# kartikmadhira1/YA_VO

Hardware: AMD Instinct MI355X
Metric: frames/sec (detect+describe+match+PnP) on 1241×376 KITTI stereo; RMSE vs CPU ref (higher is better)
Workload: dtype u8

## Files before the change

include/yavo/yavo.h:

```cpp
#ifndef YAVO_H
#define YAVO_H

#include <stddef.h>
#include <stdint.h>

#include "yavo_types.h"

#ifdef __cplusplus
extern "C" {
#endif

#define YV_OK 0
#define YV_ERR_INVALID (-1)
#define YV_ERR_HIP (-2)
#define YV_ERR_NODEVICE (-3)
#define YV_ERR_CAPACITY (-4)

#define YV_ABI_VERSION 2

typedef struct yv_ctx yv_ctx;
typedef struct yv_batch yv_batch;

int yv_abi_version(void);
const char* yv_status_string(int status);
// ... 73 lines not shown
int yv_batch_orient_view_get(yv_batch* b, yv_batch_orient_view* v);
int yv_batch_set_match_gates(yv_batch* b, const int32_t* gates , int n_pairs);
int yv_batch_set_stereo_subpix(yv_batch* b, const int32_t* pair_idx , int n, int half_win, int search,
                               int flags);
typedef struct yv_batch_subpix_view {
    const int32_t* dcol_q8;
    const int32_t* sad;
    const uint8_t* status;
} yv_batch_subpix_view;
int yv_batch_subpix_view_get(yv_batch* b, yv_batch_subpix_view* v);
int yv_batch_set_tracks(yv_batch* b, const int32_t* tracks , int n_tracks, const double K[9],
                        const double T_right[7]);
int yv_batch_track(yv_batch* b, const double* d_priors, double* d_poses, void* stream);
int yv_batch_set_track_overlap(yv_batch* b, int on);
int yv_batch_track_sync(yv_batch* b);
int yv_batch_set_track_lk(yv_batch* b, int image_step, int win, int max_level, int max_count, double eps,
                          double min_eig);
int yv_batch_enable_timing(yv_batch* b, int on);
int yv_batch_stage_times(yv_batch* b, float* ms , int* n_runs);
#define YV_NUM_STAGES 7

typedef struct yv_batch_view {
    int max_images, max_kp, max_pairs, H, W;
    int64_t cand_cap;
    const uint32_t* cand_count;
    const int32_t* det_count;
    const int32_t* det_rc;
    const float* det_resp;
    const int32_t* kp_count;
    const yv_keypoint* keypoints;
// ... 26 lines not shown
```

ya_vo_amd/__init__.py:

```python
from __future__ import annotations

import atexit
import ctypes
import os
import weakref
from typing import Optional, Tuple

import numpy as np

_HERE = os.path.dirname(os.path.abspath(__file__))
LIB_PATH = os.environ.get("YAVO_LIB") or os.path.join(_HERE, "lib", "libyavo.so")

YV_OK = 0
YV_ERR_INVALID = -1
YV_ERR_HIP = -2
YV_ERR_NODEVICE = -3
YV_ERR_CAPACITY = -4
YV_NUM_STAGES = 7
STAGE_NAMES = ("detect", "topk", "brief", "match", "finalize", "track_edges", "track_pose")

KEYPOINT_DTYPE = np.dtype([("x", "<i4"), ("y", "<i4"), ("id", "<i4"), ("matched", "u1"),
                           ("featVec", "u1", (32,)), ("_pad", "u1", (3,))])
MATCH_DTYPE = np.dtype([("pt1", KEYPOINT_DTYPE), ("pt2", KEYPOINT_DTYPE), ("distance", "<i4")])
assert KEYPOINT_DTYPE.itemsize == 48 and MATCH_DTYPE.itemsize == 100
# ... 77 lines not shown
    "yv_batch_orient_view_get": (_I, [_P, ctypes.POINTER(_BatchOrientView)]),
    "yv_stereo_subpix": (_I, [_P, _P, _P, _I, _I, _I, _P, _I, _I, _I, _P, _P, _P]),
    "yv_batch_set_stereo_subpix": (_I, [_P, _P, _I, _I, _I, _I]),
    "yv_batch_subpix_view_get": (_I, [_P, ctypes.POINTER(_BatchSubpixView)]),
    "yv_batch_create": (_I, [_P, _I, _I, _I, _I, _I, ctypes.POINTER(_P)]),
    "yv_batch_destroy": (None, [_P]),
    "yv_batch_set_pairs": (_I, [_P, _P, _I]),
    "yv_batch_run": (_I, [_P, _P, _I, _I, ctypes.c_int64, _I, _I, _P]),
    "yv_batch_enable_timing": (_I, [_P, _I]),
    "yv_batch_stage_times": (_I, [_P, _P, ctypes.POINTER(_I)]),
    "yv_batch_view_get": (_I, [_P, ctypes.POINTER(_BatchView)]),
    "yv_batch_set_tracks": (_I, [_P, _P, _I, _P, _P]),
    "yv_batch_track": (_I, [_P, _P, _P, _P]),
    "yv_batch_set_track_overlap": (_I, [_P, _I]),
    "yv_batch_track_sync": (_I, [_P]),
    "yv_batch_set_track_lk": (_I, [_P, _I, _I, _I, _I, ctypes.c_double, ctypes.c_double]),
}


_D = ctypes.c_double
GEOM_SIGNATURES = {
    "yv_f_ransac": (_I, [_P, _P, _I, _P, _I, _D, _P, ctypes.POINTER(_I), ctypes.POINTER(_I)]),
    "yv_triangulate": (_I, [_P, _P, _P, _P, _P, _I, _P, _P, ctypes.POINTER(_I)]),
    "yv_triangulate_subpix": (_I, [_P, _P, _P, _P, _P, _P, _I, _P, _P, ctypes.POINTER(_I)]),
    "yv_world2camera": (_I, [_P, _P, _I, _P, _P, _P]),
    "yv_pose_lm": (_I, [_P, _P, _P, _I, _P, _P, _P, ctypes.POINTER(_I)]),
    "yv_pose_gn": (_I, [_P, _P, _P, _I, _P, _P, ctypes.POINTER(_I)]),
    "yv_pose_lm_batch": (_I, [_P, _I, _P, _P, _P, _P, _P, _P, _P, _P]),
    "yv_pose_gn_batch": (_I, [_P, _I, _P, _P, _P, _P, _P, _P, _P]),
    "yv_f_ransac_batch": (_I, [_P, _P, ctypes.c_int64, _P, _I, _P, ctypes.c_int64, _I, _D, _P, _P, _P, _P]),
# ... 518 lines not shown
    def map_release(self, stream: int) -> None:
        _check(self.lib.yv_batch_map_release(self.handle, ctypes.c_void_p(stream)), "yv_batch_map_release")

    def set_track_overlap(self, on=True) -> None:
        mode = int(on) if not isinstance(on, bool) else (1 if on else 0)
        _check(self.lib.yv_batch_set_track_overlap(self.handle, mode), "yv_batch_set_track_overlap")

    def set_track_lk(self, image_step: int, win: int = 11, max_level: int = 3, max_count: int = 30, eps: float = 0.01,
                     min_eig: float = 0.001) -> None:
        _check(self.lib.yv_batch_set_track_lk(self.handle, image_step, win, max_level, max_count, eps, min_eig),
               "yv_batch_set_track_lk")

    def track_sync(self) -> None:
        _check(self.lib.yv_batch_track_sync(self.handle), "yv_batch_track_sync")

    def enable_timing(self, on=True) -> None:
        mode = 2 if (not isinstance(on, bool) and on == 2) else (1 if on else 0)
        _check(self.lib.yv_batch_enable_timing(self.handle, mode), "yv_batch_enable_timing")

    def stage_times(self) -> Tuple[np.ndarray, int]:
        ms = np.zeros(8, np.float32)
        n = ctypes.c_int()
        _check(self.lib.yv_batch_stage_times(self.handle, _ptr(ms), ctypes.byref(n)), "yv_batch_stage_times")
        return ms[:YV_NUM_STAGES].copy(), n.value

    def view(self) -> _BatchView:
        v = _BatchView()
        _check(self.lib.yv_batch_view_get(self.handle, ctypes.byref(v)), "yv_batch_view_get")
        return v

# ... 266 lines not shown
```

ya_vo_amd/csrc/yavo_api.hip:

```cpp
#include "yavo_host.h"

using namespace yavo;

namespace {

bool in_pinned_scratch(const yv_ctx* ctx, const void* p) {
    const char* c = static_cast<const char*>(p);
    const char* b = reinterpret_cast<const char*>(ctx->h_pinned);
    return ctx->h_pinned && c >= b && c < b + 64 * sizeof(int32_t);
}

}

namespace yavo {

int ctx_device(yv_ctx* ctx) { return ctx->device; }
hipStream_t ctx_stream(yv_ctx* ctx) { return ctx->stream; }

hipError_t stage_sync(yv_ctx* ctx, hipStream_t s) {
    hipError_t e = hipStreamSynchronize(s);
    if (e != hipSuccess) {
        ctx->pending.clear();
        return e;
    }
// ... 154 lines not shown
static int ctx_cus(yv_ctx* ctx) {
    if (ctx->cus <= 0) {
        int cus = 0;
        if (hipDeviceGetAttribute(&cus, hipDeviceAttributeMultiprocessorCount, ctx->device) != hipSuccess || cus <= 0) {
            (void)hipGetLastError();
            cus = 256;
        }
        ctx->cus = cus;
    }
    return ctx->cus;
}

int brief_workers(yv_ctx* ctx, int W) {
    const int w = ctx_cus(ctx) * yavo::brief_workers_per_cu(W);
    return ctx->brief_cap > 0 ? std::min(w, ctx->brief_cap) : w;
}

}

namespace {

int ensure_single(yv_ctx* ctx, int H, int W) {
    if (ctx->single && ctx->single->H == H && ctx->single->W == W) return YV_OK;
    if (ctx->single) {
        batch_free(ctx->single);
        ctx->single = nullptr;
    }
    yv_batch* b = nullptr;
    int rc = yv_batch_create(ctx, 1, H, W, yavo::kMaxKp, 1, &b);
    if (rc != YV_OK) return rc;
// ... 113 lines not shown
    (void)hipSetDevice(ctx->device);
    if (ctx->stream) (void)hipStreamSynchronize(ctx->stream);
    if (ctx->lk_cache) yv_lk_destroy(ctx->lk_cache);
    if (ctx->ess_cache) yv_essential_destroy(ctx->ess_cache);
    batch_free(ctx->single);
    if (ctx->side) (void)hipStreamSynchronize(ctx->side);
    delete ctx;
}

void* yv_stream(yv_ctx* ctx) { return ctx ? reinterpret_cast<void*>(ctx->stream) : nullptr; }

void* yv_side_stream(yv_ctx* ctx) {
    if (!ctx) return nullptr;
    if (ctx->side) return reinterpret_cast<void*>(ctx->side);
    if (set_device(ctx) != YV_OK) return nullptr;
    const int cus = ctx_cus(ctx);
    std::vector<uint32_t> mask((size_t)(cus + 31) / 32, 0u);
    for (int c = 0; c < cus; ++c) mask[(size_t)c / 32] |= 1u << (c % 32);
    if (hipExtStreamCreateWithCUMask(&ctx->side, (uint32_t)mask.size(), mask.data()) != hipSuccess) {
        ctx->side = nullptr;
        (void)hipGetLastError();
        if (hipStreamCreateWithFlags(&ctx->side, hipStreamNonBlocking) != hipSuccess) ctx->side = nullptr;
    }
    if (ctx->side) ctx->mem.adopt(ctx->side);
    return reinterpret_cast<void*>(ctx->side);
}

int yv_sync(yv_ctx* ctx) {
    if (!ctx) return YV_ERR_INVALID;
    YV_HIP(hipStreamSynchronize(ctx->stream));
    return YV_OK;
}

int yv_download(yv_ctx* ctx, void* host_dst, const void* dev_src, size_t bytes) {
    if (!ctx || (bytes > 0 && (!host_dst || !dev_src))) return YV_ERR_INVALID;
    if (bytes == 0) return YV_OK;
    if (set_device(ctx) != YV_OK) return YV_ERR_HIP;
    YV_HIP(hipMemcpyAsync(host_dst, dev_src, bytes, hipMemcpyDeviceToHost, ctx->stream));
// ... 405 lines not shown
```

ya_vo_amd/csrc/yavo_batch.hip:

```cpp
#include "yavo_host.h"

using namespace yavo;

namespace {

constexpr int kMaxTimedRuns = 4096;

int upload_pairs_rev(yv_batch* b) {
    if (!b->m2_alloc || b->n_pairs <= 0) return YV_OK;
    std::vector<int32_t> r(b->h_pairs.size());
    for (size_t i = 0; i + 1 < r.size(); i += 2) {
        r[i] = b->h_pairs[i + 1];
        r[i + 1] = b->h_pairs[i];
    }
    YV_HIP(hipMemcpyAsync(b->pairs_rev, r.data(), sizeof(int32_t) * r.size(), hipMemcpyHostToDevice, b->ctx->stream));
    YV_HIP(hipStreamSynchronize(b->ctx->stream));
    return YV_OK;
}

int record_stage(yv_batch* b, hipStream_t s, int run, int stage) {
    if (!b->timing || run < 0) return YV_OK;
    if (b->timing == 2 && stage > 1) return YV_OK;
    YV_HIP(hipEventRecord(b->events[(size_t)run * kEvPerRun + stage], s));
    return YV_OK;
}

yavo::MatchLists match_lists(const yv_batch* b) { return {b->desc, b->keypoints, b->kp_count, b->max_kp}; }

yavo::MatchRecords match_records(const yv_batch* b) {
    return {b->matches, b->match_count, b->filtered, b->filt_count, b->match_dj, b->match_lim};
}

static_assert(YV_SUBPIX_NONE == yavo::kSubpixNone && YV_SUBPIX_OK == yavo::kSubpixOk &&
                  YV_SUBPIX_OUTSIDE == yavo::kSubpixOutside && YV_SUBPIX_EDGE == yavo::kSubpixEdge,
              "yavo.h / yavo_internal.h");

int subpix_fill_none(yv_batch* b, hipStream_t s) {
    const size_t n = (size_t)std::max(b->max_pairs, 1) * (size_t)b->max_kp;
    YV_HIP(hipMemsetAsync(b->subpix_dcol, 0, n * sizeof(int32_t), s));
    YV_HIP(hipMemsetAsync(b->subpix_sad, 0xFF, n * sizeof(int32_t), s));
    YV_HIP(hipMemsetAsync(b->subpix_status, YV_SUBPIX_NONE, n, s));
    return YV_OK;
}

int ensure_subpix(yv_batch* b) {
// ... 8 lines not shown
        b->mem.release(b->subpix_pairs, b->subpix_dcol, b->subpix_sad, b->subpix_status);
        return YV_ERR_HIP;
    }
    b->subpix_alloc = true;
    return YV_OK;
}

}

namespace yavo {

void batch_free(yv_batch* b) {
    if (!b) return;
    if (b->bstream) (void)hipStreamSynchronize(b->bstream);
    if (b->side) (void)hipStreamSynchronize(b->side);
    if (b->lk) yv_lk_destroy(b->lk);
    delete b;
}

static_assert(YV_MATCH_RATIO == yavo::kMatchRatio && YV_MATCH_MUTUAL == yavo::kMatchMutual, "yavo.h / yavo_internal.h");
static_assert(sizeof(yv_match2) == sizeof(int4), "nn2 is written as int4 {d1, j1, d2, j2}");

bool match_filter_args_ok(int flags, int num, int den) {
    if (flags < 0 || flags > (YV_MATCH_RATIO | YV_MATCH_MUTUAL)) return false;
    if ((flags & YV_MATCH_RATIO) && !(num > 0 && num <= den && den <= 32768)) return false;
    return true;
}

int ensure_match2(yv_batch* b) {
    if (b->m2_alloc) return YV_OK;
// ... 126 lines not shown
    uint32_t* key2 = st.top2 ? b->match_key2 : nullptr;
    if (st.gated) {
        yavo::launch_gate_sort(b->keypoints, b->kp_count, b->nslots, b->max_kp, b->gate_bands, b->gate_cols,
                               b->gate_shift, b->gate_sorted, b->gate_band, s);
        yavo::launch_match_gated(lists, b->pairs, st.n_pairs, b->gate_bands, b->gate_sorted, b->gate_band, b->gates,
                                 false, b->match_key, key2, s);
        if (st.with_rev)
            yavo::launch_match_gated(lists, b->pairs_rev, st.n_pairs, b->gate_bands, b->gate_sorted, b->gate_band,
                                     b->gates, true, b->rev_key, nullptr, s);
    } else {
        yavo::launch_match(lists, b->pairs, st.n_pairs, st.max_train, b->match_key, key2, s);
        if (st.with_rev) yavo::launch_match(lists, b->pairs_rev, st.n_pairs, st.max_train_rev, b->rev_key, nullptr, s);
    }
    const int rc = record_stage(b, s, run, 4);
    const yavo::FinalizeRobust rb{b->match_key2, b->rev_key, st.flags, st.num, st.den, b->nn2, b->rev, b->keep};
    yavo::launch_match_finalize(b->match_key, lists, b->pairs, st.n_pairs, st.thr, match_records(b),
                                st.top2 ? &rb : nullptr, s, st.kp_count_copy, st.n_slots);
    return rc;
}

}

extern "C" {

int yv_batch_create(yv_ctx* ctx, int max_images, int H, int W, int max_kp, int max_pairs, yv_batch** out) {
    if (!ctx || !out || max_images <= 0 || H < 9 || W < 9 || max_kp <= 0 || max_kp > yavo::kMaxKp ||
        max_pairs < 0 || (int64_t)H * W >= (1ll << 31))
        return YV_ERR_INVALID;
    if (W > yavo::kMaxWidth) return YV_ERR_CAPACITY;
    if (H > yavo::kBandRows * yavo::kMaxBands) return YV_ERR_CAPACITY;
    *out = nullptr;
    if (set_device(ctx) != YV_OK) return YV_ERR_HIP;
// ... 59 lines not shown

void yv_batch_destroy(yv_batch* b) {
    if (!b) return;
    (void)hipSetDevice(b->ctx->device);
    (void)hipStreamSynchronize(b->ctx->stream);
    batch_free(b);
}

int yv_batch_set_pairs(yv_batch* b, const int32_t* pairs, int n_pairs) {
    if (!b || n_pairs < 0 || n_pairs > b->max_pairs || (n_pairs > 0 && !pairs)) return YV_ERR_INVALID;
    for (int i = 0; i < 2 * n_pairs; ++i)
        if (pairs[i] < 0 || pairs[i] > b->max_images) return YV_ERR_INVALID;
    if (set_device(b->ctx) != YV_OK) return YV_ERR_HIP;
    if (b->bstream) YV_HIP(hipStreamSynchronize(b->bstream));
    b->build_pending = false;
    if (n_pairs > 0) {
        YV_HIP(hipMemcpyAsync(b->pairs, pairs, sizeof(int32_t) * 2 * (size_t)n_pairs, hipMemcpyHostToDevice,
                              b->ctx->stream));
        YV_HIP(hipStreamSynchronize(b->ctx->stream));
    }
    b->h_pairs.assign(pairs, pairs + 2 * (size_t)n_pairs);
    b->n_pairs = n_pairs;
    b->n_tracks = 0;
    b->gated = false;
    b->subpix_on = false;
    return upload_pairs_rev(b);
}

int yv_batch_set_stereo_subpix(yv_batch* b, const int32_t* pair_idx, int n, int half_win, int search, int flags) {
    if (!b || n < 0) return YV_ERR_INVALID;
// ... 132 lines not shown

int yv_batch_run(yv_batch* b, const uint8_t* d_images, int n_images, int stride, int64_t image_pitch, int match_thr,
                 int carry_from, void* stream) {
    if (!b || !d_images || n_images <= 0 || n_images > b->max_images || stride < b->W ||
        image_pitch < (int64_t)stride * (b->H - 1) + b->W || carry_from >= n_images)
        return YV_ERR_INVALID;
    yv_ctx* ctx = b->ctx;
    if (set_device(ctx) != YV_OK) return YV_ERR_HIP;
    hipStream_t s = stream ? reinterpret_cast<hipStream_t>(stream) : ctx->stream;
    const int H = b->H, W = b->W, K = b->max_kp;
    const int keep = std::min(ctx->max_corners, K);
    const int sel = prepare_select(b, H, W);
    if (sel != YV_OK) return sel;
    const bool steer = steer_on(ctx);
    if (steer && ensure_steer(b) != YV_OK) return YV_ERR_HIP;
    if (b->pending_carry >= 0 && join_build(b, s) != YV_OK) return YV_ERR_HIP;
    if (b->pending_carry >= 0) {
        const size_t c = (size_t)b->pending_carry, dst = (size_t)b->max_images, nk = (size_t)K;
        YV_HIP(hipMemcpyAsync(b->keypoints + dst * nk, b->keypoints + c * nk, nk * sizeof(yv_keypoint),
                              hipMemcpyDeviceToDevice, s));
        YV_HIP(hipMemcpyAsync(b->desc + dst * nk, b->desc + c * nk, nk * sizeof(Desc), hipMemcpyDeviceToDevice, s));
        YV_HIP(hipMemcpyAsync(b->kp_count + dst, b->kp_count + c, sizeof(int32_t), hipMemcpyDeviceToDevice, s));
        if (steer) {
            YV_HIP(hipMemcpyAsync(b->steer_bin + dst * nk, b->steer_bin + c * nk, nk, hipMemcpyDeviceToDevice, s));
            YV_HIP(hipMemcpyAsync(b->steer_mom + dst * nk * 2, b->steer_mom + c * nk * 2, nk * 2 * sizeof(int32_t),
                                  hipMemcpyDeviceToDevice, s));
        }
        b->pending_carry = -1;
    }
    int run = -1;
    if (b->timing && b->runs_recorded < kMaxTimedRuns) run = b->runs_recorded++;
    b->last_run = run;
    int rc = YV_OK;
    rc |= record_stage(b, s, run, 0);
    yavo::launch_detect_blur(d_images, n_images, H, W, stride, image_pitch, ctx->fast_thr, ctx->harris_eigen, b->cand_keys, b->cap,
                             b->cand_count, ctx->k9, b->blur, s);
    rc |= record_stage(b, s, run, 1);
    if (b->overlap_mode == 2) rc |= launch_deferred_after(b, s);
    launch_select_topk(b, n_images, keep, s);
    rc |= record_stage(b, s, run, 2);
    if (b->overlap_mode == 4) rc |= launch_deferred_after(b, s);
    rc |= join_build(b, s);
    launch_describe(b, n_images, brief_workers(ctx, W), s);
    rc |= record_stage(b, s, run, 3);
    if (b->overlap_mode == 3) rc |= launch_deferred_after(b, s);
    b->run_flags = b->n_pairs > 0 ? b->match_flags : 0;
    const bool copy_counts = b->n_pairs > 0 && b->overlap && b->build_async && b->lk_step == 0;
    if (b->n_pairs > 0) {
        MatchStage st;
        st.n_pairs = b->n_pairs;
        st.max_train = st.max_train_rev = K;
        st.top2 = b->run_flags != 0;
        st.with_rev = st.top2 && (b->match_flags & YV_MATCH_MUTUAL) != 0;
        st.gated = b->gated;
        st.thr = match_thr;
        st.flags = b->match_flags;
        st.num = b->ratio_num;
        st.den = b->ratio_den;
        st.kp_count_copy = copy_counts ? b->kp_count_build : nullptr;
        st.n_slots = b->nslots;
        rc |= match_stage(b, st, s, run);
        if (b->subpix_on)
            yavo::launch_subpix_batch(d_images, n_images, H, W, stride, image_pitch, b->subpix_pairs, b->subpix_n,
                                      b->pairs, b->keypoints, b->kp_count, b->match_dj, b->match_lim,
                                      b->run_flags ? b->keep : nullptr, K, b->subpix_win, b->subpix_search,
                                      yavo::SubpixOut{b->subpix_dcol, b->subpix_sad, b->subpix_status}, s);
    } else {
        rc |= record_stage(b, s, run, 4);
    }
    b->counts_copied = copy_counts;
    rc |= record_stage(b, s, run, 5);
    if (rc != YV_OK) return YV_ERR_HIP;
    b->pending_carry = carry_from;
    b->run_images = d_images;
    b->run_n = n_images;
// ... 40 lines not shown
```

ya_vo_amd/csrc/yavo_batch_track.hip:

```cpp
#include "yavo_host.h"

#include <cstdlib>

#include "../../include/yavo/yavo_map.h"

using namespace yavo;

namespace yavo {

int join_build(yv_batch* b, hipStream_t s) {
    if (!b->build_pending) return YV_OK;
    YV_HIP(hipStreamWaitEvent(s, b->ev_built, 0));
    b->build_pending = false;
    return YV_OK;
}

EdgeSlice edge_slice(const yv_batch* b, int k) {
    if (!b->edge_X) return {};
    const size_t nt = (size_t)b->max_tracks, nk = (size_t)b->max_kp;
    return {b->edge_X + k * nt * nk * 3, b->edge_uv + k * nt * nk * 2,  b->edge_query + k * nt * nk,
            b->edge_count + k * nt,      b->edge_outlier + k * nt * nk, b->track_inliers + k * nt};
}

}

namespace {

TrackSrc track_src(const yv_batch* b) {
// ... 146 lines not shown
            const int prev = b->h_pairs[2 * sp];
            if (prev % b->lk_step || prev >= b->max_images || tp < 0 || tp >= b->max_images || tp % b->lk_step)
                return YV_ERR_INVALID;
        } else {
            if (tp < 0 || tp >= b->n_pairs) return YV_ERR_INVALID;
            if (b->h_pairs[2 * sp] != b->h_pairs[2 * tp + 1]) return YV_ERR_INVALID;
        }
    }
    for (int i = 0; i < 9 && n_tracks > 0; ++i)
        if (!std::isfinite(K[i])) return YV_ERR_INVALID;
    if (n_tracks > 0 && !finite_pose(T_right)) return YV_ERR_INVALID;
    if (set_device(b->ctx) != YV_OK) return YV_ERR_HIP;
    hipStream_t s = b->ctx->stream;
    if (b->bstream) YV_HIP(hipStreamSynchronize(b->bstream));
    b->build_pending = false;
    if (b->side) YV_HIP(hipStreamSynchronize(b->side));
    if (n_tracks > b->max_tracks) {
        YV_HIP(hipStreamSynchronize(s));
        if (b->side) YV_HIP(hipStreamSynchronize(b->side));
        b->track_mem.clear();
        b->max_tracks = 0;
        b->n_tracks = 0;
        const size_t nt = (size_t)n_tracks, nk = (size_t)b->max_kp;
        int rc = YV_OK;
        rc |= b->track_mem.alloc(&b->tracks, 2 * nt);
        rc |= b->track_mem.alloc(&b->track_K, 9 * nt);
        rc |= b->track_mem.alloc(&b->T_right, 7);
        rc |= b->track_mem.alloc(&b->edge_X, kEdgeBufs * 3 * nt * nk);
        rc |= b->track_mem.alloc(&b->edge_uv, kEdgeBufs * 2 * nt * nk);
        rc |= b->track_mem.alloc(&b->edge_query, kEdgeBufs * nt * nk);
// ... 70 lines not shown
    if (set_device(b->ctx) != YV_OK) return YV_ERR_HIP;
    if (flush_deferred(b) != YV_OK) return YV_ERR_HIP;
    if (on && !b->side) {
        int least = 0, greatest = 0;
        YV_HIP(hipDeviceGetStreamPriorityRange(&least, &greatest));
        YV_HIP(hipStreamCreateWithPriority(&b->side, hipStreamNonBlocking, least));
        b->mem.adopt(b->side);
        for (int k = 0; k < kEdgeBufs; ++k) {
            YV_HIP(b->mem.event(&b->ev_edges[k]));
            YV_HIP(b->mem.event(&b->ev_lm[k]));
        }
        YV_HIP(hipStreamCreateWithFlags(&b->bstream, hipStreamNonBlocking));
        b->mem.adopt(b->bstream);
        YV_HIP(b->mem.event(&b->ev_fin));
        YV_HIP(b->mem.event(&b->ev_built));
    }
    if (!on && b->bstream) YV_HIP(hipStreamSynchronize(b->bstream));
    if (!on) b->build_pending = false;
    {
        const char* e = std::getenv("YAVO_BUILD_ASYNC");
        b->build_async = on != 0 && !(e && e[0] == '0');
    }
    if (!on && b->side) YV_HIP(hipStreamSynchronize(b->side));
    b->overlap = on != 0;
    b->overlap_mode = on;
    return YV_OK;
}

int yv_batch_track_sync(yv_batch* b) {
    if (!b) return YV_ERR_INVALID;
    if (set_device(b->ctx) != YV_OK) return YV_ERR_HIP;
    if (flush_deferred(b) != YV_OK) return YV_ERR_HIP;
    if (b->bstream) YV_HIP(hipStreamSynchronize(b->bstream));
    if (b->side) YV_HIP(hipStreamSynchronize(b->side));
    return YV_OK;
}

int yv_batch_set_track_lk(yv_batch* b, int image_step, int win, int max_level, int max_count, double eps,
                          double min_eig) {
    if (!b || image_step < 0 || (image_step > 0 && (win < 3 || win > 22 || max_level < 0))) return YV_ERR_INVALID;
    if (set_device(b->ctx) != YV_OK) return YV_ERR_HIP;
    if (flush_deferred(b) != YV_OK) return YV_ERR_HIP;
    if (b->side) YV_HIP(hipStreamSynchronize(b->side));
    if (b->bstream) YV_HIP(hipStreamSynchronize(b->bstream));
    b->build_pending = false;
    YV_HIP(hipStreamSynchronize(b->ctx->stream));
    if (b->lk) {
        yv_lk_destroy(b->lk);
        b->lk = nullptr;
    }
    b->lk_step = image_step;
    b->n_tracks = 0;
    if (image_step == 0) return YV_OK;
    const int slots = (b->max_images + image_step - 1) / image_step;
    const int rc = yv_lk_create(b->ctx, slots, b->H, b->W, win, max_level, &b->lk);
    if (rc != YV_OK) {
        b->lk_step = 0;
        return rc;
    }
    b->lk_max_count = max_count;
// ... 7 lines not shown
```

ya_vo_amd/csrc/yavo_host.h:

```cpp
#pragma once

#include <hip/hip_runtime.h>

#include <algorithm>
#include <cmath>
#include <cstdio>
#include <cstring>
#include <new>
#include <vector>

#include "../../include/yavo/yavo.h"
#include "yavo_internal.h"

#define YV_HIP(call)                                                                           \
    do {                                                                                       \
        hipError_t e_ = (call);                                                                \
        if (e_ != hipSuccess) {                                                                \
            std::fprintf(stderr, "yavo: %s failed: %s (%s:%d)\n", #call, hipGetErrorString(e_), \
                         __FILE__, __LINE__);                                                  \
            return YV_ERR_HIP;                                                                 \
        }                                                                                      \
    } while (0)

namespace yavo {
// ... 241 lines not shown
    int overlap_mode = 0;
    struct DeferredLM {
        bool active = false;
        int k = 0, run = -1;
        const double* priors = nullptr;
        double* poses = nullptr;
        hipEvent_t* ev = nullptr;
        bool has_map = false;
        yavo::MapArgs map;
    } deferred;
    hipEvent_t ev_defer = nullptr;
    hipStream_t side = nullptr;
    hipStream_t bstream = nullptr;
    bool build_async = false, build_pending = false;
    hipEvent_t ev_fin = nullptr, ev_built = nullptr;
    hipEvent_t ev_edges[kEdgeBufs] = {}, ev_lm[kEdgeBufs] = {};
    bool lm_pending[kEdgeBufs] = {};
    hipEvent_t ev_map = nullptr;
    bool map_written = false;
    hipEvent_t ev_map_release = nullptr;
    bool map_release_pending = false;
    int timing = 0;
    std::vector<hipEvent_t> events;
    std::vector<uint8_t> tracked;
    int runs_recorded = 0;
    int last_run = -1;
    int pending_carry = -1;
};

namespace yavo {

inline int set_device(yv_ctx* ctx) {
    YV_HIP(hipSetDevice(ctx->device));
    return YV_OK;
}

inline bool select_on(const yv_ctx* ctx) { return ctx->sel_radius > 0 || ctx->sel_q > 0; }
inline bool steer_on(const yv_ctx* ctx) { return ctx->steer_bins > 0; }

int brief_workers(yv_ctx* ctx, int W);

hipError_t stage_sync(yv_ctx* ctx, hipStream_t s);
uint8_t* stage_alloc(yv_ctx* ctx, size_t bytes, hipStream_t s);
hipError_t stage_h2d(yv_ctx* ctx, void* dst, const void* src, size_t bytes, hipStream_t s);
hipError_t stage_h2d_2d(yv_ctx* ctx, void* dst, size_t dpitch, const void* src, size_t spitch, size_t width,
                        size_t height, hipStream_t s);
hipError_t stage_d2h(yv_ctx* ctx, void* dst, const void* src, size_t bytes, hipStream_t s);

struct StageScope {
    yv_ctx* ctx;
    explicit StageScope(yv_ctx* c) : ctx(c) {}
    ~StageScope() { ctx->pending.clear(); }
};

struct Arena {
// ... 32 lines not shown
    hipError_t download(hipStream_t s);
    void finish();
    hipError_t fetch(hipStream_t s);
};

struct MatchStage {
    int n_pairs = 1;
    int max_train = 0, max_train_rev = 0;
    bool top2 = false;
    bool with_rev = false;
    bool gated = false;
    int thr = 0;
    int flags = 0, num = 0, den = 1;
    int32_t* kp_count_copy = nullptr;
    int n_slots = 0;
};

void batch_free(yv_batch* b);
bool match_filter_args_ok(int flags, int num, int den);
bool gate_ok(const int32_t* g);
bool select_fits(const yv_ctx* ctx, int H, int W);
int ensure_match2(yv_batch* b);
int ensure_gates(yv_batch* b, int max_row, int max_col);
int ensure_steer(yv_batch* b);
int prepare_select(yv_batch* b, int H, int W);
void launch_select_topk(yv_batch* b, int n_images, int keep, hipStream_t s);
void launch_describe(yv_batch* b, int n_images, int max_workers, hipStream_t s);
int match_stage(yv_batch* b, MatchStage st, hipStream_t s, int run);

constexpr int kEvPerRun = 9;
int join_build(yv_batch* b, hipStream_t s);
int launch_deferred_after(yv_batch* b, hipStream_t s);
struct EdgeSlice {
    double* X;
    double* uv;
    int32_t* query;
    int32_t* count;
    uint8_t* outlier;
    int32_t* inliers;
};
EdgeSlice edge_slice(const yv_batch* b, int k);

}
```

ya_vo_amd/csrc/yavo_internal.h:

```cpp
#pragma once

#include <hip/hip_runtime.h>
#include <stdint.h>

#include "../../include/yavo/yavo_types.h"

struct yv_ctx;

namespace yavo {

__host__ __device__ inline double cube_cr(double t) {
    const double p = t * t, e1 = fma(t, t, -p);
    const double q = p * t, e2 = fma(p, t, -q);
    return q + (e2 + e1 * t);
}

constexpr int kMaxKp = 4096;
constexpr int kMaxWidth = 2048;
constexpr int kBandRows = 32;
constexpr int kMaxBands = 256;
constexpr int kBandCounters = 1024;
constexpr int kFastTileW = 64;
constexpr int kFastTileH = 56;
__host__ __device__ constexpr int blur_pitch(int W) { return (W + 1 + 127) & ~127; }
// ... 35 lines not shown
void launch_pack_desc(const yv_keypoint* keypoints, const int32_t* kp_count, int n_slots, int max_kp,
                      Desc* desc, hipStream_t s);
struct MatchLists {
    const Desc* desc;
    const yv_keypoint* keypoints;
    const int32_t* kp_count;
    int max_kp;
};
struct MatchRecords {
    yv_match* matches;
    int32_t* match_count;
    yv_match* filtered;
    int32_t* filt_count;
    int2* match_dj;
    int32_t* match_lim;
};
void launch_match(const MatchLists& lists, const int32_t* pairs, int n_pairs, int max_train, uint32_t* match_key,
                  uint32_t* match_key2, hipStream_t s);
constexpr int kMatchRatio = 1, kMatchMutual = 2;
struct FinalizeRobust {
    uint32_t* match_key2;
    uint32_t* rev_key;
    int flags, num, den;
    int4* nn2;
    int32_t* rev;
    uint8_t* keep;
};
void launch_match_finalize(uint32_t* match_key, const MatchLists& lists, const int32_t* pairs, int n_pairs, int thr,
                           const MatchRecords& out, const FinalizeRobust* rb, hipStream_t s,
                           int32_t* kp_count_copy = nullptr, int n_slots = 0);
constexpr int kGateBandRows = 32;
constexpr int kGateMaxCells = 8192;
constexpr int kGateMaxCoord = 65535;
void launch_gate_sort(const yv_keypoint* keypoints, const int32_t* kp_count, int n_slots, int max_kp, int n_bands,
                      int col_cells, int col_shift, uint2* sorted, int32_t* band_start, hipStream_t s);
void launch_match_gated(const MatchLists& lists, const int32_t* pairs, int n_pairs, int n_bands, const uint2* sorted,
                        const int32_t* band_start, const int32_t* gates, bool mirror, uint32_t* match_key,
                        uint32_t* match_key2, hipStream_t s);
constexpr int kSelMaxCells = 8192;
constexpr int kSelTileRows = 32, kSelTileCols = 64;
constexpr int kSelMaxRadius = 8;
constexpr int kSelMaxPerCell = 4096;
constexpr int kSelMinCell = 8, kSelMaxCell = 8192;
uint32_t* launch_select(uint64_t* cand_keys, int64_t cap, uint32_t* cand_count, uint32_t* cand_seen, int n_images,
                        int H, int W, int nms_radius, int cell_rows, int cell_cols, int per_cell, uint64_t* scratch,
// ... 215 lines not shown
```

ya_vo_amd/csrc/yavo_kernels.hip:

```cpp
#include <hip/hip_runtime.h>
#include <stdint.h>
#include <stdlib.h>
#include <string.h>

#include <algorithm>

#include "yavo_xlane.h"
#include "yavo_internal.h"


namespace yavo {

__device__ __forceinline__ int lane_id() { return (int)(threadIdx.x & 63); }

__device__ __forceinline__ int wave_incl_scan(int v) {
    v += __builtin_amdgcn_update_dpp(0, v, 0x111, 0xf, 0xf, false);
    v += __builtin_amdgcn_update_dpp(0, v, 0x112, 0xf, 0xf, false);
    v += __builtin_amdgcn_update_dpp(0, v, 0x114, 0xf, 0xf, false);
    v += __builtin_amdgcn_update_dpp(0, v, 0x118, 0xf, 0xf, false);
    v += __builtin_amdgcn_update_dpp(0, v, 0x142, 0xa, 0xf, false);
    v += __builtin_amdgcn_update_dpp(0, v, 0x143, 0xc, 0xf, false);
    return v;
}

// ... 1468 lines not shown
    for (int off = 32; off > 0; off >>= 1) v = min(v, __shfl_xor(v, off, 64));
    const int wave = (int)threadIdx.x >> 6;
    if (lane_id() == 0) s_tmp[wave] = v;
    __syncthreads();
    int r = s_tmp[0];
    for (int w = 1; w < (int)(blockDim.x >> 6); ++w) r = min(r, s_tmp[w]);
    __syncthreads();
    return r;
}

__device__ __forceinline__ int outlier_limit(int min_d, int thr) {
    const int twice = (int)((uint32_t)min_d * 2u);
    return twice > thr ? twice : thr;
}

template <bool ROBUST>
__global__ __launch_bounds__(FZ_NT) void match_finalize_kernel(
    uint32_t* __restrict__ match_key, const yv_keypoint* __restrict__ keypoints,
    const int32_t* __restrict__ kp_count, const int32_t* __restrict__ pairs, int max_kp, int thr,
    yv_match* __restrict__ matches, int32_t* __restrict__ match_count, yv_match* __restrict__ filtered,
    int32_t* __restrict__ filt_count, int2* __restrict__ match_dj, int32_t* __restrict__ match_lim,
    int32_t* __restrict__ kp_count_copy, int n_slots, FinalizeRobust rb) {
    __shared__ int s_dist[kMaxKp];
    if (kp_count_copy && blockIdx.x == 0)
        for (int i = (int)threadIdx.x; i < n_slots; i += FZ_NT) kp_count_copy[i] = kp_count[i];
    __shared__ int s_j[kMaxKp];
    __shared__ int s_pos[kMaxKp];
    __shared__ int s_tmp[40];
    const int pair = blockIdx.x;
    const int tid = threadIdx.x;
    const int qi = pairs[2 * pair], ti = pairs[2 * pair + 1];
    const int nq = kp_count[qi];
    uint32_t* keys = match_key + (int64_t)pair * max_kp;
    int local_min = 0x7fffffff;
    for (int i = tid; i < nq; i += FZ_NT) {
        const uint32_t k = keys[i];
        keys[i] = 0xFFFFFFFFu;
// ... 37 lines not shown
        flags[u] = (i < nq && s_dist[i] < lim) ? 1 : 0;
        if constexpr (ROBUST) {
            if (i < nq) {
                flags[u] &= s_pos[i];
                rb.keep[(int64_t)pair * max_kp + i] = (uint8_t)flags[u];
            }
        }
        cnt += flags[u];
        if (i < nq) dj[i] = make_int2(s_dist[i], s_j[i]);
    }
    int total = 0;
    int off = block_excl_scan<FZ_NT>(cnt, s_tmp, &total);
#pragma unroll
    for (int u = 0; u < 4; ++u) {
        const int i = tid * 4 + u;
        if (i < nq) s_pos[i] = flags[u] ? off : -1;
        off += flags[u];
    }
    __syncthreads();
    const uint32_t* qrec = reinterpret_cast<const uint32_t*>(keypoints + (int64_t)qi * max_kp);
    const uint32_t* trec = reinterpret_cast<const uint32_t*>(keypoints + (int64_t)ti * max_kp);
    uint32_t* out_all = reinterpret_cast<uint32_t*>(matches + (int64_t)pair * max_kp);
    uint32_t* out_f = reinterpret_cast<uint32_t*>(filtered + (int64_t)pair * max_kp);
    const int ndw = nq * REC_DW;
    constexpr int FZ_U = 4;
    for (int dw0 = tid; dw0 < ndw; dw0 += FZ_U * FZ_NT) {
        uint32_t v[FZ_U];
        int ii[FZ_U], ff[FZ_U];
#pragma unroll
        for (int u = 0; u < FZ_U; ++u) {
            const int dw = min(dw0 + u * FZ_NT, ndw - 1);
            const int i = dw / REC_DW, f = dw - i * REC_DW;
            const int j = s_j[i];
            const uint32_t* src = f < 12 ? qrec + (int64_t)i * 12 + f : trec + (int64_t)max(j, 0) * 12 + min(f - 12, 2);
            v[u] = *src;
            ii[u] = i;
            ff[u] = f;
        }
#pragma unroll
        for (int u = 0; u < FZ_U; ++u) {
            const int dw = dw0 + u * FZ_NT;
            if (dw >= ndw) break;
            const int i = ii[u], f = ff[u];
            uint32_t x = v[u];
            if (f == 11) x &= 0xFFu;
            else if (f >= 12 && (f >= 15 || s_j[i] < 0)) x = 0;
            if (f == 24) x = (uint32_t)s_dist[i];
            out_all[dw] = x;
            const int p = s_pos[i];
            if (p >= 0) {
                if (f == 3 || f == 15) x = (x & ~0xFFu) | 1u;
                out_f[(int64_t)p * REC_DW + f] = x;
            }
        }
    }
    if (tid == 0) {
        match_count[pair] = nq;
        filt_count[pair] = total;
        match_lim[pair] = lim;
    }
}

void launch_match_finalize(uint32_t* match_key, const MatchLists& lists, const int32_t* pairs, int n_pairs, int thr,
                           const MatchRecords& out, const FinalizeRobust* rb, hipStream_t s, int32_t* kp_count_copy,
                           int n_slots) {
    const auto kernel = !rb ? match_finalize_kernel<false> : match_finalize_kernel<true>;
    hipLaunchKernelGGL(kernel, dim3(n_pairs), dim3(FZ_NT), 0, s, match_key, lists.keypoints, lists.kp_count, pairs,
                       lists.max_kp, thr, out.matches, out.match_count, out.filtered, out.filt_count, out.match_dj,
                       out.match_lim, kp_count_copy, n_slots, rb ? *rb : FinalizeRobust{});
}

__global__ __launch_bounds__(FZ_NT) void filter_records_kernel(const yv_match* __restrict__ in, int n, int thr,
                                                               yv_match* __restrict__ out,
                                                               int32_t* __restrict__ out_count) {
    __shared__ int s_pos[kMaxKp];
    __shared__ int s_tmp[40];
    const int tid = threadIdx.x;
    const uint32_t* src = reinterpret_cast<const uint32_t*>(in);
    int local_min = 0x7fffffff;
    for (int i = tid; i < n; i += FZ_NT) local_min = min(local_min, (int)src[(int64_t)i * REC_DW + 24]);
    const int min_d = block_min_int(local_min, s_tmp);
    const int lim = outlier_limit(min_d, thr);
    int flags[4], cnt = 0;
#pragma unroll
// ... 69 lines not shown
```

Baseline: 254,400.

## Defer match record materialization to a separate stream overlapping tracking

Splits match finalize so that, when tracking is enabled and async build/overlap is on, the kernel only writes per-query filtered positions. A new match_records kernel on a dedicated CU-masked stream then writes the full and filtered 100-byte match records, using LDS staging and nontemporal vector stores. Later consumers (next run, track sync, set_pairs) wait on an event or drain the stream. The aim is to take the record-writing traffic off the critical path and let it overlap with tracking. The cost is an extra stream, an extra match_pos buffer and added synchronization complexity.

```diff
diff --git a/include/yavo/yavo.h b/include/yavo/yavo.h
--- a/include/yavo/yavo.h
+++ b/include/yavo/yavo.h
@@ -111,6 +111,7 @@
 int yv_batch_track(yv_batch* b, const double* d_priors, double* d_poses, void* stream);
 int yv_batch_set_track_overlap(yv_batch* b, int on);
 int yv_batch_track_sync(yv_batch* b);
+int yv_batch_records_wait(yv_batch* b, void* stream);
 int yv_batch_set_track_lk(yv_batch* b, int image_step, int win, int max_level, int max_count, double eps,
                           double min_eig);
 int yv_batch_enable_timing(yv_batch* b, int on);
diff --git a/ya_vo_amd/__init__.py b/ya_vo_amd/__init__.py
--- a/ya_vo_amd/__init__.py
+++ b/ya_vo_amd/__init__.py
@@ -115,6 +115,7 @@
     "yv_batch_track": (_I, [_P, _P, _P, _P]),
     "yv_batch_set_track_overlap": (_I, [_P, _I]),
     "yv_batch_track_sync": (_I, [_P]),
+    "yv_batch_records_wait": (_I, [_P, _P]),
     "yv_batch_set_track_lk": (_I, [_P, _I, _I, _I, _I, ctypes.c_double, ctypes.c_double]),
 }
 
@@ -663,6 +664,9 @@
     def track_sync(self) -> None:
         _check(self.lib.yv_batch_track_sync(self.handle), "yv_batch_track_sync")
 
+    def records_wait(self, stream: int) -> None:
+        _check(self.lib.yv_batch_records_wait(self.handle, ctypes.c_void_p(stream)), "yv_batch_records_wait")
+
     def enable_timing(self, on=True) -> None:
         mode = 2 if (not isinstance(on, bool) and on == 2) else (1 if on else 0)
         _check(self.lib.yv_batch_enable_timing(self.handle, mode), "yv_batch_enable_timing")
diff --git a/ya_vo_amd/csrc/yavo_api.hip b/ya_vo_amd/csrc/yavo_api.hip
--- a/ya_vo_amd/csrc/yavo_api.hip
+++ b/ya_vo_amd/csrc/yavo_api.hip
@@ -192,6 +192,21 @@
 int brief_workers(yv_ctx* ctx, int W) {
     const int w = ctx_cus(ctx) * yavo::brief_workers_per_cu(W);
     return ctx->brief_cap > 0 ? std::min(w, ctx->brief_cap) : w;
+}
+
+int records_workgroups(yv_ctx* ctx) { return ctx_cus(ctx) * 8; }
+
+hipStream_t make_queue_stream(yv_ctx* ctx) {
+    const int cus = ctx_cus(ctx);
+    std::vector<uint32_t> mask((size_t)(cus + 31) / 32, 0u);
+    for (int c = 0; c < cus; ++c) mask[(size_t)c / 32] |= 1u << (c % 32);
+    hipStream_t s = nullptr;
+    if (hipExtStreamCreateWithCUMask(&s, (uint32_t)mask.size(), mask.data()) != hipSuccess) {
+        s = nullptr;
+        (void)hipGetLastError();
+        if (hipStreamCreateWithFlags(&s, hipStreamNonBlocking) != hipSuccess) s = nullptr;
+    }
+    return s;
 }
 
 }
@@ -335,14 +350,7 @@
     if (!ctx) return nullptr;
     if (ctx->side) return reinterpret_cast<void*>(ctx->side);
     if (set_device(ctx) != YV_OK) return nullptr;
-    const int cus = ctx_cus(ctx);
-    std::vector<uint32_t> mask((size_t)(cus + 31) / 32, 0u);
-    for (int c = 0; c < cus; ++c) mask[(size_t)c / 32] |= 1u << (c % 32);
-    if (hipExtStreamCreateWithCUMask(&ctx->side, (uint32_t)mask.size(), mask.data()) != hipSuccess) {
-        ctx->side = nullptr;
-        (void)hipGetLastError();
-        if (hipStreamCreateWithFlags(&ctx->side, hipStreamNonBlocking) != hipSuccess) ctx->side = nullptr;
-    }
+    ctx->side = make_queue_stream(ctx);
     if (ctx->side) ctx->mem.adopt(ctx->side);
     return reinterpret_cast<void*>(ctx->side);
 }
diff --git a/ya_vo_amd/csrc/yavo_batch.hip b/ya_vo_amd/csrc/yavo_batch.hip
--- a/ya_vo_amd/csrc/yavo_batch.hip
+++ b/ya_vo_amd/csrc/yavo_batch.hip
@@ -27,8 +27,14 @@
 
 yavo::MatchLists match_lists(const yv_batch* b) { return {b->desc, b->keypoints, b->kp_count, b->max_kp}; }
 
-yavo::MatchRecords match_records(const yv_batch* b) {
-    return {b->matches, b->match_count, b->filtered, b->filt_count, b->match_dj, b->match_lim};
+yavo::MatchRecords match_records(const yv_batch* b, bool deferred) {
+    return {b->matches,  b->match_count, b->filtered, b->filt_count,
+            b->match_dj, b->match_lim,   deferred ? b->match_pos : nullptr};
+}
+
+int ensure_match_pos(yv_batch* b) {
+    if (b->match_pos) return YV_OK;
+    return b->mem.alloc(&b->match_pos, (size_t)std::max(b->max_pairs, 1) * (size_t)b->max_kp);
 }
 
 static_assert(YV_SUBPIX_NONE == yavo::kSubpixNone && YV_SUBPIX_OK == yavo::kSubpixOk &&
@@ -67,6 +73,7 @@
     if (!b) return;
     if (b->bstream) (void)hipStreamSynchronize(b->bstream);
     if (b->side) (void)hipStreamSynchronize(b->side);
+    if (b->rstream) (void)hipStreamSynchronize(b->rstream);
     if (b->lk) yv_lk_destroy(b->lk);
     delete b;
 }
@@ -223,8 +230,17 @@
     }
     const int rc = record_stage(b, s, run, 4);
     const yavo::FinalizeRobust rb{b->match_key2, b->rev_key, st.flags, st.num, st.den, b->nn2, b->rev, b->keep};
-    yavo::launch_match_finalize(b->match_key, lists, b->pairs, st.n_pairs, st.thr, match_records(b),
-                                st.top2 ? &rb : nullptr, s, st.kp_count_copy, st.n_slots);
+    const yavo::MatchRecords out = match_records(b, st.defer_records);
+    yavo::launch_match_finalize(b->match_key, lists, b->pairs, st.n_pairs, st.thr, out, st.top2 ? &rb : nullptr, s,
+                                st.kp_count_copy, st.n_slots);
+    if (st.defer_records) {
+        YV_HIP(hipEventRecord(b->ev_keys, s));
+        YV_HIP(hipStreamWaitEvent(b->rstream, b->ev_keys, 0));
+        yavo::launch_match_records({lists.desc, lists.keypoints, st.kp_count_copy, lists.max_kp}, b->pairs, st.n_pairs,
+                                   out, records_workgroups(b->ctx), b->rstream);
+        YV_HIP(hipEventRecord(b->ev_records, b->rstream));
+        b->records_pending = true;
+    }
     return rc;
 }
 
@@ -314,6 +330,7 @@
     if (set_device(b->ctx) != YV_OK) return YV_ERR_HIP;
     if (b->bstream) YV_HIP(hipStreamSynchronize(b->bstream));
     b->build_pending = false;
+    if (drain_records(b) != YV_OK) return YV_ERR_HIP;
     if (n_pairs > 0) {
         YV_HIP(hipMemcpyAsync(b->pairs, pairs, sizeof(int32_t) * 2 * (size_t)n_pairs, hipMemcpyHostToDevice,
                               b->ctx->stream));
@@ -476,7 +493,9 @@
     if (sel != YV_OK) return sel;
     const bool steer = steer_on(ctx);
     if (steer && ensure_steer(b) != YV_OK) return YV_ERR_HIP;
-    if (b->pending_carry >= 0 && join_build(b, s) != YV_OK) return YV_ERR_HIP;
+    const bool defer_records = b->rstream && b->n_tracks > 0 && b->timing != 1;
+    if (defer_records && ensure_match_pos(b) != YV_OK) return YV_ERR_HIP;
+    if (b->pending_carry >= 0 && (join_build(b, s) != YV_OK || join_records(b, s) != YV_OK)) return YV_ERR_HIP;
     if (b->pending_carry >= 0) {
         const size_t c = (size_t)b->pending_carry, dst = (size_t)b->max_images, nk = (size_t)K;
         YV_HIP(hipMemcpyAsync(b->keypoints + dst * nk, b->keypoints + c * nk, nk * sizeof(yv_keypoint),
@@ -503,11 +522,13 @@
     rc |= record_stage(b, s, run, 2);
     if (b->overlap_mode == 4) rc |= launch_deferred_after(b, s);
     rc |= join_build(b, s);
+    rc |= join_records(b, s);
     launch_describe(b, n_images, brief_workers(ctx, W), s);
     rc |= record_stage(b, s, run, 3);
     if (b->overlap_mode == 3) rc |= launch_deferred_after(b, s);
     b->run_flags = b->n_pairs > 0 ? b->match_flags : 0;
     const bool copy_counts = b->n_pairs > 0 && b->overlap && b->build_async && b->lk_step == 0;
+    const bool defer = copy_counts && defer_records;
     if (b->n_pairs > 0) {
         MatchStage st;
         st.n_pairs = b->n_pairs;
@@ -521,6 +542,7 @@
         st.den = b->ratio_den;
         st.kp_count_copy = copy_counts ? b->kp_count_build : nullptr;
         st.n_slots = b->nslots;
+        st.defer_records = defer;
         rc |= match_stage(b, st, s, run);
         if (b->subpix_on)
             yavo::launch_subpix_batch(d_images, n_images, H, W, stride, image_pitch, b->subpix_pairs, b->subpix_n,
diff --git a/ya_vo_amd/csrc/yavo_batch_track.hip b/ya_vo_amd/csrc/yavo_batch_track.hip
--- a/ya_vo_amd/csrc/yavo_batch_track.hip
+++ b/ya_vo_amd/csrc/yavo_batch_track.hip
@@ -12,6 +12,19 @@
     if (!b->build_pending) return YV_OK;
     YV_HIP(hipStreamWaitEvent(s, b->ev_built, 0));
     b->build_pending = false;
+    return YV_OK;
+}
+
+int join_records(yv_batch* b, hipStream_t s) {
+    if (!b->records_pending) return YV_OK;
+    YV_HIP(hipStreamWaitEvent(s, b->ev_records, 0));
+    b->records_pending = false;
+    return YV_OK;
+}
+
+int drain_records(yv_batch* b) {
+    if (b->rstream) YV_HIP(hipStreamSynchronize(b->rstream));
+    b->records_pending = false;
     return YV_OK;
 }
 
@@ -188,6 +201,7 @@
     hipStream_t s = b->ctx->stream;
     if (b->bstream) YV_HIP(hipStreamSynchronize(b->bstream));
     b->build_pending = false;
+    if (drain_records(b) != YV_OK) return YV_ERR_HIP;
     if (b->side) YV_HIP(hipStreamSynchronize(b->side));
     if (n_tracks > b->max_tracks) {
         YV_HIP(hipStreamSynchronize(s));
@@ -288,9 +302,15 @@
         b->mem.adopt(b->bstream);
         YV_HIP(b->mem.event(&b->ev_fin));
         YV_HIP(b->mem.event(&b->ev_built));
+        b->rstream = make_queue_stream(b->ctx);
+        if (!b->rstream) return YV_ERR_HIP;
+        b->mem.adopt(b->rstream);
+        YV_HIP(b->mem.event(&b->ev_keys));
+        YV_HIP(b->mem.event(&b->ev_records));
     }
     if (!on && b->bstream) YV_HIP(hipStreamSynchronize(b->bstream));
     if (!on) b->build_pending = false;
+    if (!on && drain_records(b) != YV_OK) return YV_ERR_HIP;
     {
         const char* e = std::getenv("YAVO_BUILD_ASYNC");
         b->build_async = on != 0 && !(e && e[0] == '0');
@@ -307,6 +327,13 @@
     if (flush_deferred(b) != YV_OK) return YV_ERR_HIP;
     if (b->bstream) YV_HIP(hipStreamSynchronize(b->bstream));
     if (b->side) YV_HIP(hipStreamSynchronize(b->side));
+    return drain_records(b);
+}
+
+int yv_batch_records_wait(yv_batch* b, void* stream) {
+    if (!b || !stream) return YV_ERR_INVALID;
+    if (set_device(b->ctx) != YV_OK) return YV_ERR_HIP;
+    if (b->records_pending) YV_HIP(hipStreamWaitEvent(reinterpret_cast<hipStream_t>(stream), b->ev_records, 0));
     return YV_OK;
 }
 
@@ -318,6 +345,7 @@
     if (b->side) YV_HIP(hipStreamSynchronize(b->side));
     if (b->bstream) YV_HIP(hipStreamSynchronize(b->bstream));
     b->build_pending = false;
+    if (drain_records(b) != YV_OK) return YV_ERR_HIP;
     YV_HIP(hipStreamSynchronize(b->ctx->stream));
     if (b->lk) {
         yv_lk_destroy(b->lk);
diff --git a/ya_vo_amd/csrc/yavo_host.h b/ya_vo_amd/csrc/yavo_host.h
--- a/ya_vo_amd/csrc/yavo_host.h
+++ b/ya_vo_amd/csrc/yavo_host.h
@@ -279,6 +279,10 @@
     hipStream_t bstream = nullptr;
     bool build_async = false, build_pending = false;
     hipEvent_t ev_fin = nullptr, ev_built = nullptr;
+    hipStream_t rstream = nullptr;
+    hipEvent_t ev_keys = nullptr, ev_records = nullptr;
+    bool records_pending = false;
+    int32_t* match_pos = nullptr;
     hipEvent_t ev_edges[kEdgeBufs] = {}, ev_lm[kEdgeBufs] = {};
     bool lm_pending[kEdgeBufs] = {};
     hipEvent_t ev_map = nullptr;
@@ -304,6 +308,8 @@
 inline bool steer_on(const yv_ctx* ctx) { return ctx->steer_bins > 0; }
 
 int brief_workers(yv_ctx* ctx, int W);
+int records_workgroups(yv_ctx* ctx);
+hipStream_t make_queue_stream(yv_ctx* ctx);
 
 hipError_t stage_sync(yv_ctx* ctx, hipStream_t s);
 uint8_t* stage_alloc(yv_ctx* ctx, size_t bytes, hipStream_t s);
@@ -366,6 +372,7 @@
     int flags = 0, num = 0, den = 1;
     int32_t* kp_count_copy = nullptr;
     int n_slots = 0;
+    bool defer_records = false;
 };
 
 void batch_free(yv_batch* b);
@@ -382,6 +389,8 @@
 
 constexpr int kEvPerRun = 9;
 int join_build(yv_batch* b, hipStream_t s);
+int join_records(yv_batch* b, hipStream_t s);
+int drain_records(yv_batch* b);
 int launch_deferred_after(yv_batch* b, hipStream_t s);
 struct EdgeSlice {
     double* X;
diff --git a/ya_vo_amd/csrc/yavo_internal.h b/ya_vo_amd/csrc/yavo_internal.h
--- a/ya_vo_amd/csrc/yavo_internal.h
+++ b/ya_vo_amd/csrc/yavo_internal.h
@@ -73,6 +73,7 @@
     int32_t* filt_count;
     int2* match_dj;
     int32_t* match_lim;
+    int32_t* match_pos;
 };
 void launch_match(const MatchLists& lists, const int32_t* pairs, int n_pairs, int max_train, uint32_t* match_key,
                   uint32_t* match_key2, hipStream_t s);
@@ -88,6 +89,8 @@
 void launch_match_finalize(uint32_t* match_key, const MatchLists& lists, const int32_t* pairs, int n_pairs, int thr,
                            const MatchRecords& out, const FinalizeRobust* rb, hipStream_t s,
                            int32_t* kp_count_copy = nullptr, int n_slots = 0);
+void launch_match_records(const MatchLists& lists, const int32_t* pairs, int n_pairs, const MatchRecords& out,
+                          int max_workgroups, hipStream_t s);
 constexpr int kGateBandRows = 32;
 constexpr int kGateMaxCells = 8192;
 constexpr int kGateMaxCoord = 65535;
diff --git a/ya_vo_amd/csrc/yavo_kernels.hip b/ya_vo_amd/csrc/yavo_kernels.hip
--- a/ya_vo_amd/csrc/yavo_kernels.hip
+++ b/ya_vo_amd/csrc/yavo_kernels.hip
@@ -1506,13 +1506,27 @@
     return twice > thr ? twice : thr;
 }
 
-template <bool ROBUST>
+__device__ __forceinline__ int record_train_dword(int f) { return min(f - 12, 2); }
+__device__ __forceinline__ const uint32_t* record_src(const uint32_t* qrec, const uint32_t* trec, int i, int j, int f) {
+    return f < 12 ? qrec + (int64_t)i * 12 + f : trec + (int64_t)max(j, 0) * 12 + record_train_dword(f);
+}
+__device__ __forceinline__ uint32_t record_dword(uint32_t x, int f, int j, int dist) {
+    if (f == 11) x &= 0xFFu;
+    else if (f >= 12 && (f >= 15 || j < 0)) x = 0;
+    if (f == 24) x = (uint32_t)dist;
+    return x;
+}
+__device__ __forceinline__ uint32_t record_dword_kept(uint32_t x, int f) {
+    return (f == 3 || f == 15) ? (x & ~0xFFu) | 1u : x;
+}
+
+template <bool ROBUST, bool RECORDS>
 __global__ __launch_bounds__(FZ_NT) void match_finalize_kernel(
     uint32_t* __restrict__ match_key, const yv_keypoint* __restrict__ keypoints,
     const int32_t* __restrict__ kp_count, const int32_t* __restrict__ pairs, int max_kp, int thr,
     yv_match* __restrict__ matches, int32_t* __restrict__ match_count, yv_match* __restrict__ filtered,
     int32_t* __restrict__ filt_count, int2* __restrict__ match_dj, int32_t* __restrict__ match_lim,
-    int32_t* __restrict__ kp_count_copy, int n_slots, FinalizeRobust rb) {
+    int32_t* __restrict__ match_pos, int32_t* __restrict__ kp_count_copy, int n_slots, FinalizeRobust rb) {
     __shared__ int s_dist[kMaxKp];
     if (kp_count_copy && blockIdx.x == 0)
         for (int i = (int)threadIdx.x; i < n_slots; i += FZ_NT) kp_count_copy[i] = kp_count[i];
@@ -1580,43 +1594,41 @@
 #pragma unroll
     for (int u = 0; u < 4; ++u) {
         const int i = tid * 4 + u;
-        if (i < nq) s_pos[i] = flags[u] ? off : -1;
+        if constexpr (RECORDS) {
+            if (i < nq) s_pos[i] = flags[u] ? off : -1;
+        } else {
+            if (i < nq) match_pos[(int64_t)pair * max_kp + i] = flags[u] ? off : -1;
+        }
         off += flags[u];
     }
-    __syncthreads();
-    const uint32_t* qrec = reinterpret_cast<const uint32_t*>(keypoints + (int64_t)qi * max_kp);
-    const uint32_t* trec = reinterpret_cast<const uint32_t*>(keypoints + (int64_t)ti * max_kp);
-    uint32_t* out_all = reinterpret_cast<uint32_t*>(matches + (int64_t)pair * max_kp);
-    uint32_t* out_f = reinterpret_cast<uint32_t*>(filtered + (int64_t)pair * max_kp);
-    const int ndw = nq * REC_DW;
-    constexpr int FZ_U = 4;
-    for (int dw0 = tid; dw0 < ndw; dw0 += FZ_U * FZ_NT) {
-        uint32_t v[FZ_U];
-        int ii[FZ_U], ff[FZ_U];
-#pragma unroll
-        for (int u = 0; u < FZ_U; ++u) {
-            const int dw = min(dw0 + u * FZ_NT, ndw - 1);
-            const int i = dw / REC_DW, f = dw - i * REC_DW;
-            const int j = s_j[i];
-            const uint32_t* src = f < 12 ? qrec + (int64_t)i * 12 + f : trec + (int64_t)max(j, 0) * 12 + min(f - 12, 2);
-            v[u] = *src;
-            ii[u] = i;
-            ff[u] = f;
-        }
-#pragma unroll
-        for (int u = 0; u < FZ_U; ++u) {
-            const int dw = dw0 + u * FZ_NT;
-            if (dw >= ndw) break;
-            const int i = ii[u], f = ff[u];
-            uint32_t x = v[u];
-            if (f == 11) x &= 0xFFu;
-            else if (f >= 12 && (f >= 15 || s_j[i] < 0)) x = 0;
-            if (f == 24) x = (uint32_t)s_dist[i];
-            out_all[dw] = x;
-            const int p = s_pos[i];
-            if (p >= 0) {
-                if (f == 3 || f == 15) x = (x & ~0xFFu) | 1u;
-                out_f[(int64_t)p * REC_DW + f] = x;
+    if constexpr (RECORDS) {
+        __syncthreads();
+        const uint32_t* qrec = reinterpret_cast<const uint32_t*>(keypoints + (int64_t)qi * max_kp);
+        const uint32_t* trec = reinterpret_cast<const uint32_t*>(keypoints + (int64_t)ti * max_kp);
+        uint32_t* out_all = reinterpret_cast<uint32_t*>(matches + (int64_t)pair * max_kp);
+        uint32_t* out_f = reinterpret_cast<uint32_t*>(filtered + (int64_t)pair * max_kp);
+        const int ndw = nq * REC_DW;
+        constexpr int FZ_U = 4;
+        for (int dw0 = tid; dw0 < ndw; dw0 += FZ_U * FZ_NT) {
+            uint32_t v[FZ_U];
+            int ii[FZ_U], ff[FZ_U];
+#pragma unroll
+            for (int u = 0; u < FZ_U; ++u) {
+                const int dw = min(dw0 + u * FZ_NT, ndw - 1);
+                const int i = dw / REC_DW, f = dw - i * REC_DW;
+                v[u] = *record_src(qrec, trec, i, s_j[i], f);
+                ii[u] = i;
+                ff[u] = f;
+            }
+#pragma unroll
+            for (int u = 0; u < FZ_U; ++u) {
+                const int dw = dw0 + u * FZ_NT;
+                if (dw >= ndw) break;
+                const int i = ii[u], f = ff[u];
+                const uint32_t x = record_dword(v[u], f, s_j[i], s_dist[i]);
+                out_all[dw] = x;
+                const int p = s_pos[i];
+                if (p >= 0) out_f[(int64_t)p * REC_DW + f] = record_dword_kept(x, f);
             }
         }
     }
@@ -1627,13 +1639,91 @@
     }
 }
 
+constexpr int MR_NT = 64;
+typedef uint32_t v4u __attribute__((ext_vector_type(4)));
+
+__global__ __launch_bounds__(MR_NT) void match_records_kernel(
+    const int2* __restrict__ match_dj, const int32_t* __restrict__ match_pos,
+    const yv_keypoint* __restrict__ keypoints, const int32_t* __restrict__ kp_count,
+    const int32_t* __restrict__ pairs, int n_pairs, int max_kp, yv_match* __restrict__ matches,
+    yv_match* __restrict__ filtered) {
+    static_assert(sizeof(yv_keypoint) == 48 && sizeof(yv_match) == 4 * REC_DW, "record layout");
+    __shared__ __attribute__((aligned(16))) uint32_t s_rec[MR_NT * REC_DW];
+    const int lane = threadIdx.x;
+    const int groups = (max_kp + MR_NT - 1) / MR_NT;
+    for (int c = blockIdx.x; c < n_pairs * groups; c += gridDim.x) {
+        const int pair = c / groups, i0 = (c - pair * groups) * MR_NT;
+        const int qi = pairs[2 * pair], ti = pairs[2 * pair + 1];
+        const int nq = min(kp_count[qi], max_kp);
+        if (i0 >= nq) continue;
+        const int n = min(MR_NT, nq - i0);
+        const int i = min(i0 + lane, nq - 1);
+        const int2 d = match_dj[(int64_t)pair * max_kp + i];
+        const int p = lane < n ? match_pos[(int64_t)pair * max_kp + i] : -1;
+        uint32_t q[12], t[3];
+        const uint4* q4 = reinterpret_cast<const uint4*>(keypoints + (int64_t)qi * max_kp + i);
+#pragma unroll
+        for (int k = 0; k < 3; ++k) {
+            const uint4 w = q4[k];
+            q[4 * k] = w.x, q[4 * k + 1] = w.y, q[4 * k + 2] = w.z, q[4 * k + 3] = w.w;
+        }
+        const uint32_t* tr = reinterpret_cast<const uint32_t*>(keypoints + (int64_t)ti * max_kp + max(d.y, 0));
+#pragma unroll
+        for (int k = 0; k < 3; ++k) t[k] = tr[k];
+#pragma unroll
+        for (int f = 0; f < REC_DW; ++f)
+            s_rec[lane * REC_DW + f] = record_dword(f < 12 ? q[f] : t[record_train_dword(f)], f, d.y, d.x);
+        __syncthreads();
+        uint32_t* out_all = reinterpret_cast<uint32_t*>(matches + (int64_t)pair * max_kp + i0);
+        const int ndw = n * REC_DW;
+        if ((reinterpret_cast<uintptr_t>(out_all) & 15) == 0) {
+            for (int k = lane; 4 * k < ndw; k += MR_NT) {
+                if (4 * k + 4 <= ndw) {
+                    const uint4 w = reinterpret_cast<const uint4*>(s_rec)[k];
+                    __builtin_nontemporal_store(v4u{w.x, w.y, w.z, w.w}, reinterpret_cast<v4u*>(out_all) + k);
+                } else {
+                    for (int e = 4 * k; e < ndw; ++e) out_all[e] = s_rec[e];
+                }
+            }
+        } else {
+            for (int k = lane; k < ndw; k += MR_NT) __builtin_nontemporal_store(s_rec[k], out_all + k);
+        }
+        __syncthreads();
+        const uint64_t kept = __ballot(p >= 0);
+        if (kept != 0) {
+            const int p0 = __shfl(p, __ffsll((unsigned long long)kept) - 1);
+            if (p >= 0) {
+#pragma unroll
+                for (int f = 0; f < REC_DW; ++f)
+                    s_rec[(p - p0) * REC_DW + f] = record_dword_kept(
+                        record_dword(f < 12 ? q[f] : t[record_train_dword(f)], f, d.y, d.x), f);
+            }
+            __syncthreads();
+            uint32_t* out_f = reinterpret_cast<uint32_t*>(filtered + (int64_t)pair * max_kp + p0);
+            const int nf = __popcll(kept) * REC_DW;
+            for (int k = lane; k < nf; k += MR_NT) __builtin_nontemporal_store(s_rec[k], out_f + k);
+            __syncthreads();
+        }
+    }
+}
+
 void launch_match_finalize(uint32_t* match_key, const MatchLists& lists, const int32_t* pairs, int n_pairs, int thr,
                            const MatchRecords& out, const FinalizeRobust* rb, hipStream_t s, int32_t* kp_count_copy,
                            int n_slots) {
-    const auto kernel = !rb ? match_finalize_kernel<false> : match_finalize_kernel<true>;
+    const bool rec = out.match_pos == nullptr;
+    const auto kernel = !rb ? (rec ? match_finalize_kernel<false, true> : match_finalize_kernel<false, false>)
+                            : (rec ? match_finalize_kernel<true, true> : match_finalize_kernel<true, false>);
     hipLaunchKernelGGL(kernel, dim3(n_pairs), dim3(FZ_NT), 0, s, match_key, lists.keypoints, lists.kp_count, pairs,
                        lists.max_kp, thr, out.matches, out.match_count, out.filtered, out.filt_count, out.match_dj,
-                       out.match_lim, kp_count_copy, n_slots, rb ? *rb : FinalizeRobust{});
+                       out.match_lim, out.match_pos, kp_count_copy, n_slots, rb ? *rb : FinalizeRobust{});
+}
+
+void launch_match_records(const MatchLists& lists, const int32_t* pairs, int n_pairs, const MatchRecords& out,
+                          int max_workgroups, hipStream_t s) {
+    const int64_t groups = (int64_t)n_pairs * ((lists.max_kp + MR_NT - 1) / MR_NT);
+    const int grid = (int)std::min<int64_t>(groups, std::max(max_workgroups, 1));
+    hipLaunchKernelGGL(match_records_kernel, dim3(grid), dim3(MR_NT), 0, s, out.match_dj, out.match_pos,
+                       lists.keypoints, lists.kp_count, pairs, n_pairs, lists.max_kp, out.matches, out.filtered);
 }
 
 __global__ __launch_bounds__(FZ_NT) void filter_records_kernel(const yv_match* __restrict__ in, int n, int thr,
```

New measurement: 265,800 (median of 6 runs). 1.04x the previous value.
